# i8run/BigDL

Hardware: AMD Instinct MI355X
Metric: images/sec (whole node) ResNet-50 224x224 bf16 at 1/2/4/8 MI355X (higher is better)
Workload: dtype bf16; 1 GPU; model=ResNet-50 v1.5 (BigDL ImageNet builder), global_batch=256, per_gpu_batch=256, image=224, parallelism=dp1, optimizer=SGD momentum 0.9 + L2 1e-4 (one rank: no gradient exchange), hip_graph=False, wgrad_side_stream=True, bucketed_overlap=False, grad_compress=none (no exchange)

## Files before the change

### csrc/bindings.cpp

```cpp
#include <torch/extension.h>
#include <ATen/hip/HIPContext.h>
#include <vector>
#include <algorithm>
#include "kernels.h"

namespace {

using at::Tensor;
using OptT = c10::optional<Tensor>;

hipStream_t stream() { return at::hip::getCurrentHIPStream().stream(); }

void check(const Tensor& t, at::ScalarType dt, const char* name) {
  TORCH_CHECK(t.is_cuda(), name, " must be a GPU tensor");
  TORCH_CHECK(t.scalar_type() == dt, name, " has dtype ", t.scalar_type(), ", expected ", dt);
}
const uint16_t* cbf(const Tensor& t, const char* n) { check(t, at::kBFloat16, n); return (const uint16_t*)t.data_ptr(); }
uint16_t* mbf(const Tensor& t, const char* n) { check(t, at::kBFloat16, n); return (uint16_t*)t.data_ptr(); }
const float* cf(const Tensor& t, const char* n) { check(t, at::kFloat, n); return (const float*)t.data_ptr(); }
float* mf(const Tensor& t, const char* n) { check(t, at::kFloat, n); return (float*)t.data_ptr(); }
const uint16_t* ocbf(const OptT& t, const char* n) { return (t && t->defined()) ? cbf(*t, n) : nullptr; }
uint16_t* ombf(const OptT& t, const char* n) { return (t && t->defined()) ? mbf(*t, n) : nullptr; }
const float* ocf(const OptT& t, const char* n) { return (t && t->defined()) ? cf(*t, n) : nullptr; }
float* omf(const OptT& t, const char* n) { return (t && t->defined()) ? mf(*t, n) : nullptr; }
// ... 257 lines not shown
  TORCH_CHECK(geo.size() == 18, who, ": bad geometry");
  WgradArgs a{};
  int* f = &a.Nb;
  for (int i = 0; i < 18; ++i) f[i] = (int)geo[i];
  static float dummy;
  a.dbias = bias ? &dummy : nullptr;
  return bigdl_conv_wgrad_choose(&a);
}

bool conv_wgrad_uses_p8(std::vector<int64_t> geo, bool bias) {
  const int k = wgrad_choice_of(geo, bias, "conv_wgrad_uses_p8").kernel;
  return k == WGRAD_P8 || k == WGRAD_P8_DIRECT;
}

std::vector<int64_t> conv_wgrad_plan_info(std::vector<int64_t> geo, bool bias) {
  const WgradChoice c = wgrad_choice_of(geo, bias, "conv_wgrad_plan_info");
  const bool atomic = c.kernel == WGRAD_GLDS_ATOMIC || c.kernel == WGRAD_G3_ATOMIC;
  return {c.kernel == WGRAD_REG ? 0 : atomic ? 1 : c.splits, c.ws_floats, c.kernel == WGRAD_HALO ? c.splits : 0,
          c.kernel == WGRAD_P8 || c.kernel == WGRAD_P8_DIRECT, c.kernel == WGRAD_REG};
}

std::string conv_wgrad_plan_name(std::vector<int64_t> geo, bool bias) {
  return bigdl_wgrad_kernel_name(wgrad_choice_of(geo, bias, "conv_wgrad_plan_name").kernel);
}

void transpose_krsc(const Tensor& w, const Tensor& wt, int64_t K, int64_t RS, int64_t C) {
  TORCH_CHECK(w.numel() == K * RS * C && wt.numel() == K * RS * C, "transpose_krsc: size mismatch");
  bigdl_transpose_krsc(cbf(w, "w"), mbf(wt, "wt"), (int)K, (int)RS, (int)C, stream());
}

void bn_stats(const Tensor& x, const Tensor& stats, int64_t P, int64_t C) {
  TORCH_CHECK(C % 8 == 0 && x.numel() == P * C, "bn_stats: shape");
  TORCH_CHECK(stats.numel() >= BIGDL_STAT_SLOTS * 2 * C, "bn_stats: stats must hold STAT_SLOTS x 2C");
  bigdl_bn_stats(cbf(x, "x"), mf(stats, "stats"), P, (int)C, stream());
}
void bn_finalize(const Tensor& stats, int64_t nslots, const OptT& gamma, const OptT& beta, const OptT& rmean,
                 const OptT& rvar, const OptT& smean, const OptT& sinv, const Tensor& scale, const Tensor& shift,
                 int64_t P, int64_t C, double eps, double momentum, bool training) {
  TORCH_CHECK(stats.numel() >= nslots * 2 * C, "bn_finalize: stats size");
  bigdl_bn_finalize(cf(stats, "stats"), (int)nslots, ocf(gamma, "gamma"), ocf(beta, "beta"), omf(rmean, "rmean"),
                    omf(rvar, "rvar"), omf(smean, "smean"), omf(sinv, "sinv"), mf(scale, "scale"),
                    mf(shift, "shift"), P, (int)C, (float)eps, (float)momentum, training ? 1 : 0, stream());
}
void bn_slot_reduce(const Tensor& in, int64_t nslots, int64_t C, const Tensor& out) {
  TORCH_CHECK(in.numel() >= nslots * 2 * C && out.numel() >= 2 * C, "bn_slot_reduce: size");
  bigdl_bn_slot_reduce(cf(in, "in"), (int)nslots, (int)C, mf(out, "out"), stream());
// ... 1824 lines not shown
  m.def("set_conv_p8", &bigdl_set_conv_p8);
  m.def("set_conv_w8", &bigdl_set_conv_w8);
  m.def("set_wgrad_p8", &bigdl_set_wgrad_p8);
  m.def("conv_wgrad_uses_p8", &conv_wgrad_uses_p8);
  m.def("conv_wgrad_plan_info", &conv_wgrad_plan_info);
  m.def("conv_wgrad_plan_name", &conv_wgrad_plan_name);
  m.def("get_conv_shortk", &bigdl_get_conv_shortk);
  m.def("get_conv_p8", &bigdl_get_conv_p8);
  m.def("get_conv_w8", &bigdl_get_conv_w8);
  m.def("get_conv_sk", &bigdl_get_conv_sk);
  m.def("get_conv_s1", &bigdl_get_conv_s1);
  m.def("get_wgrad_p8", &bigdl_get_wgrad_p8);
  m.def("get_conv_halo", &bigdl_get_conv_halo);
  m.def("get_stem_fwd", &bigdl_get_stem_fwd);
  m.def("get_stem_wgrad", &bigdl_get_stem_wgrad);
  m.def("get_wgrad_halo", &bigdl_get_wgrad_halo);
  m.def("conv_nt_plan_info", &conv_nt_plan_info, py::arg("geo"), py::arg("taps"), py::arg("flags") = 0,
        py::arg("addend_stride") = std::vector<int64_t>());
  m.def("get_conv_g4", &bigdl_get_conv_g4);
  m.def("set_wgrad_g3", &bigdl_set_wgrad_g3);
  m.def("get_wgrad_g3", &bigdl_get_wgrad_g3);
  m.def("set_wgrad_tr_asm", &bigdl_set_wgrad_tr_asm);
  m.def("get_wgrad_tr_asm", &bigdl_get_wgrad_tr_asm);
  m.def("set_i8_g3", &bigdl_set_i8_g3);
  m.def("set_i8_p8", &bigdl_set_i8_p8);
  m.def("set_i8_s1", &bigdl_set_i8_s1);
  m.def("set_i8_epi", &bigdl_set_i8_epi);
  m.def("set_i8_shortk", &bigdl_set_i8_shortk);
  m.def("set_i8_cpl", &bigdl_set_i8_cpl);
  m.def("get_i8_g3", &bigdl_get_i8_g3);
  m.def("get_i8_p8", &bigdl_get_i8_p8);
  m.def("get_i8_s1", &bigdl_get_i8_s1);
  m.def("get_i8_epi", &bigdl_get_i8_epi);
  m.def("get_i8_shortk", &bigdl_get_i8_shortk);
  m.def("get_i8_cpl", &bigdl_get_i8_cpl);
  m.def("conv_i8_plan_info", &conv_i8_plan_info, py::arg("geo"), py::arg("taps"), py::arg("out_mode") = 0,
        py::arg("flags") = 0, py::arg("ldo_override") = 0, py::arg("add_ld") = 0,
        "(kernel, BM, BN, stages, cpl, direct, fastk) conv_i8 would run; launches nothing");
  m.attr("arch") = "gfx950";
}
```

### csrc/conv_igemm.hip

```cpp
#include "common.h"
#include "kernels.h"
#include <stdlib.h>

#include "conv_epilogue.h"
#include "lds_tr.h"


namespace {

constexpr int BK = 64;

__device__ __attribute__((aligned(64))) bf16_t g_zero_granule[32];
__device__ __forceinline__ v4u load16(const bf16_t* p, bool ok) {
  return *reinterpret_cast<const v4u*>(ok ? p : g_zero_granule);
}

template <int MI, int NI, int TM, int TN>
__device__ __forceinline__ void nt_epilogue(const ConvArgs& a, v4f (&acc)[MI][NI], int mbase, int nbase, int lane,
                                            int bid) {
  const int ohw = a.OH * a.OW;
  const bool vec_ok = (a.Ncol & 3) == 0 && (a.ldo & 3) == 0;
#pragma unroll
  for (int j = 0; j < NI; ++j) {
    const int nb = nbase + j * 16 + (lane >> 4) * 4;
// ... 2776 lines not shown
  const int tiles = ((a->Ncol + WT - 1) / WT) * ((a->Kdim + WT - 1) / WT);
  const bool dma = s.impl >= 1 && !wgrad_prefers_atomic(a);
  if (dma) {
    int splits = (s.wgrad_wgs + tiles - 1) / tiles;
    splits = std::max(1, std::min(splits, (a->M + 8 * WBM - 1) / (8 * WBM)));
    wgrad_split(&c, a->M, splits);
    if (c.splits > 1) {
      c.kernel = s.wgrad_g3 ? WGRAD_G3_WS : WGRAD_GLDS_WS;
      c.ws_floats = (long)c.splits * a->Ncol * a->Kdim;
      return c;
    }
  }
  int splits = (512 + tiles - 1) / tiles;
  const long tile_bytes = (long)tiles * WT * WT * 4;
  splits = std::min(splits, (int)(((long)s.wgrad_atomic_mb << 20) / tile_bytes));
  splits = std::min(splits, (a->M + 4 * WBM - 1) / (4 * WBM));
  if (splits < 1 || bigdl_deterministic()) splits = 1;
  wgrad_split(&c, a->M, splits);
  c.kernel = !dma ? WGRAD_REG : s.wgrad_g3 ? WGRAD_G3_ATOMIC : WGRAD_GLDS_ATOMIC;
  return c;
}

void launch_wgrad_reduce(const WgradArgs& a, int groups, hipStream_t st) {
  const long n4 = (long)a.Ncol * a.Kdim / 4;
  const int blocks = (int)std::min<long>((n4 + 255) / 256, 8192);
  if (groups < 0)
    groups = (blocks >= 256 || bigdl_deterministic()) ? 1 : std::max(1, std::min({2048 / blocks, a.splits / 4, 64}));
  const dim3 grid(blocks, groups);
  if ((reinterpret_cast<uintptr_t>(a.dw) & 15) == 0) wgrad_reduce_kernel<true><<<grid, 256, 0, st>>>(a.ws, a.dw, n4, a.splits);
  else wgrad_reduce_kernel<false><<<grid, 256, 0, st>>>(a.ws, a.dw, n4, a.splits);
}

}

extern "C" {

void bigdl_set_conv_impl(int v) { sw().impl = v; }
void bigdl_set_conv_s1(int v) { sw().s1 = v; }
void bigdl_set_conv_sk(int v) { sw().sk = v; }
void bigdl_set_conv_g4(int v) { sw().g4 = v; }
void bigdl_set_conv_shortk(int v) { sw().shortk = v; }
void bigdl_set_conv_p8(int v) { sw().p8 = v; }
void bigdl_set_conv_w8(int v) { sw().w8 = v; }
void bigdl_set_wgrad_p8(int v) { sw().wgrad_p8 = v; }
void bigdl_set_wgrad_g3(int v) { sw().wgrad_g3 = v; }
void bigdl_set_wgrad_tr_asm(int v) { sw().wgrad_tr_asm = v; }
// ... 183 lines not shown
      } else {
        if (direct) conv_wgrad_p8_kernel<true, false><<<grid, dim3(512), 0, st>>>(a);
        else conv_wgrad_p8_kernel<false, false><<<grid, dim3(512), 0, st>>>(a);
      }
      if (a.splits > 1) launch_wgrad_reduce(a, 1, st);
      break;
    }
    case WGRAD_GLDS_WS:
    case WGRAD_G3_WS:
      if (c->kernel == WGRAD_G3_WS) launch_wgrad_g3(a, tiles * spad, st);
      else launch_wgrad_glds(a, tiles * spad, st);
      launch_wgrad_reduce(a, -1, st);
      break;
    case WGRAD_GLDS_ATOMIC: launch_wgrad_glds(a, tiles * spad, st); break;
    case WGRAD_G3_ATOMIC: launch_wgrad_g3(a, tiles * spad, st); break;
    case WGRAD_REG: conv_wgrad_kernel<<<dim3(tiles, a.splits), dim3(256), 0, st>>>(a); break;
    default: return WGRAD_ERR_LAUNCH;
  }
  HIP_LAUNCH_CHECK();
  if (det_bias) bigdl_colsum_bf16_ld(a_in->dy, a_in->dbias, a_in->M, a_in->Ncol, a_in->ldy, st, a_in->det_ws);
  return 0;
}

void bigdl_transpose_krsc(const bf16_t* w, bf16_t* wt, int K, int RS, int C, hipStream_t st) {
  if (RS > 65535) return;
  if (K % 8 == 0 && C % 8 == 0 && (long)K * C >= (1L << 20) && (((uintptr_t)w | (uintptr_t)wt) & 15) == 0)
    transpose_krsc_v8_kernel<<<dim3((C + 63) / 64, (K + 63) / 64, RS), 256, 0, st>>>(w, wt, K, RS, C);
  else
    transpose_krsc_kernel<<<dim3((C + 31) / 32, (K + 31) / 32, RS), 256, 0, st>>>(w, wt, K, RS, C);
  HIP_LAUNCH_CHECK();
}

void bigdl_transpose_krsc_batched(const long* desc, int n, int total_tiles, hipStream_t st) {
  if (n <= 0 || total_tiles <= 0) return;
  transpose_krsc_batched_kernel<<<dim3(total_tiles), 256, 0, st>>>(desc, n);
  HIP_LAUNCH_CHECK();
}

}
```

### csrc/kernels.h

```cpp
#pragma once
#include <hip/hip_runtime.h>
#include <stdint.h>

#define CONV_MAX_TAPS 64
struct ConvArgs {
  const uint16_t* src;
  const uint16_t* wt;
  uint16_t* out;
  const float* bias;
  float* stats;
  const uint16_t* addend;
  const uint8_t* addzm;
  const uint16_t* bnx;
  const uint16_t* bnz;
  const uint8_t* bnzm;
  const float* bnmean;
  const float* bnaff;
  float* bnred;
  int Nb, Hs, Ws, Cs;
  int OH, OW;
  int mul_h, mul_w;
  int ntaps, ldw;
  int M, Ncol, Kdim, ldo;
  int OHo, OWo, omul_h, omul_w, ooff_h, ooff_w, ident_out;
// ... 185 lines not shown
                        const uint16_t* x2 = nullptr, const float* mean2 = nullptr, float* red2 = nullptr);

void bigdl_relu_fwd(const uint16_t* x, uint16_t* y, long n, hipStream_t st);
void bigdl_spin_us(double us, int* done, hipStream_t st);
void bigdl_dgrad_fill(uint16_t* out, const uint16_t* add, long npix, int H, int W, int C, int sh, int sw, unsigned mask,
                      hipStream_t st);
void bigdl_relu_bwd(const uint16_t* dy, const uint16_t* y, uint16_t* dx, long n, hipStream_t st);
void bigdl_add_bf16(const uint16_t* a, const uint16_t* b, uint16_t* y, long n, hipStream_t st);
void bigdl_nchw_f32_to_nhwc_bf16(const float* x, uint16_t* y, int N, int C, int H, int W, int Cp,
                                 hipStream_t st);
void bigdl_cast_f32_bf16(const float* x, uint16_t* y, long n, hipStream_t st);
void bigdl_colsum_bf16(const uint16_t* x, float* out, long P, int K, hipStream_t st, float* det_ws = nullptr);
void bigdl_ones_col_pack(const uint16_t* x, uint16_t* xe, long M, int K, hipStream_t st);
void bigdl_ones_col_acc(const float* gw, float* gW, float* gB, long N, int K, float sW, float sB, hipStream_t st);
void bigdl_cast_bf16_f32(const uint16_t* x, float* y, long n, hipStream_t st);

void bigdl_maxpool_fwd(const uint16_t* x, uint16_t* y, uint8_t* idx, int N, int H, int W, int C, int OH,
                       int OW, int kh, int kw, int sh, int sw, int ph, int pw, hipStream_t st, const float* pre = nullptr);
int bigdl_maxpool_pre_applies(int N, int H, int W, int C, int OH, int OW, int kh, int kw, int sh, int sw);
int bigdl_stem_i8_applies(const ConvArgs* a, const I8Epi* ep);
void bigdl_set_stem_i8(int v);
int bigdl_stem_i8_f32(const ConvArgs* a, const I8Epi* ep, const float* img, int C, int W, float inv, hipStream_t st);
int bigdl_stem_i8(const ConvArgs* a, const I8Epi* ep, hipStream_t st);
void bigdl_split_reduce_f32(const float* ws, float* dw, long n, int splits, hipStream_t st);
int bigdl_maxpool_bwd_bnred_applies(int N, int H, int W, int C, int OH, int OW, int kh, int kw, int sh, int sw, int ph,
                                    int pw);
void bigdl_maxpool_bwd_bnred(const uint16_t* dy, const uint8_t* idx, uint16_t* dx, int N, int C, int OH, int OW,
                             const uint16_t* bx, const float* mean, const float* aff, const uint8_t* zm, float* red,
                             hipStream_t st);
void bigdl_maxpool_bwd(const uint16_t* dy, const uint8_t* idx, uint16_t* dx, int N, int H, int W, int C,
                       int OH, int OW, int kh, int kw, int sh, int sw, int ph, int pw, hipStream_t st);
void bigdl_avgpool_fwd(const uint16_t* x, uint16_t* y, int N, int H, int W, int C, int OH, int OW, int kh,
                       int kw, int sh, int sw, int ph, int pw, int count_pad, hipStream_t st);
void bigdl_avgpool_bwd(const uint16_t* dy, uint16_t* dx, int N, int H, int W, int C, int OH, int OW, int kh,
                       int kw, int sh, int sw, int ph, int pw, int count_pad, hipStream_t st);

void bigdl_softmax_xent(const uint16_t* logits_bf16, const float* logits_f32, const float* labels,
                        float* loss, uint16_t* dlogits_bf16, float* dlogits_f32, int B, int K,
                        float label_base, float grad_scale, hipStream_t st, float* det_ws = nullptr);
#define BIGDL_XENT_SLOTS 2048

void bigdl_sgd_step(float* w, const float* g, float* mom, uint16_t* w16, long n, const float* lr_dev, float lr,
                    float wd, float momentum, double dampening, int nesterov, int first, const long* seg_off,
                    const float* seg_wd, int nseg, long base, hipStream_t st);
void bigdl_adam_step(float* w, const float* g, float* m, float* v, uint16_t* w16, long n, float lr,
                     double beta1, double beta2, float eps, float wd, float bc1, float bc2, hipStream_t st);
void bigdl_sumsq(const float* x, float* out, long n, hipStream_t st, float* det_ws = nullptr);
// ... 21 lines not shown
int bigdl_tensor_apply(float* out, const float* a, const float* b, const float* c, int nd, const long* size,
                       const long* so, const long* sa, const long* sb, const long* sc, int op, float s0, float s1,
                       int contiguous, hipStream_t st);
int bigdl_index_op(int op, float* a, const void* idx, int idx_i64, const float* b, float* out, long outer, long R,
                   long n, long inner, long Rsrc, int* err, hipStream_t st);
void bigdl_masked_fill(float* x, const float* mask, float v, long n, hipStream_t st);
long bigdl_mask_blocks(long n);
void bigdl_mask_scan(const float* mask, long n, int* counts, hipStream_t st);
void bigdl_mask_write(int copy, float* x, const float* mask, const float* src, float* out, long n, const int* counts,
                      long nsrc, hipStream_t st);
int bigdl_topk(const float* x, long outer, long R, long inner, int k, int largest, float* vals, float* inds,
               hipStream_t st);
int bigdl_tensor_reduce(const float* x, long outer, long R, long inner, int op, float p, float* out, float* outi,
                        int mean, float* ws, long chunks, hipStream_t st);
int bigdl_gemm_f32(const float* A, const float* B, const float* Min, float* C, int batch, int M, int N, int K,
                   const long* s, float alpha, float beta, hipStream_t st);
int bigdl_gemv_f32(const float* A, const float* x, const float* Min, float* y, int M, int K, long sam, long sak,
                   long sx, long smi, long sy, float alpha, float beta, hipStream_t st);
void bigdl_copy_rows_i8(const int8_t* src, int8_t* dst, long rows, int C, long lds, long ldd, hipStream_t st);
void bigdl_set_conv_impl(int impl);
void bigdl_set_conv_s1(int v);
void bigdl_set_conv_sk(int v);
void bigdl_set_wgrad_halo(int v);
int bigdl_lstm_drop_rep(const void* x, int x_bf16, long xs_b, long xs_t, uint16_t* y, long ys_g, int B, int T, int K,
                        int Kp, int ones, float p, float mul, unsigned long long seed, long long off, hipStream_t st);
int bigdl_lstm_drop_rep_bwd(const float* dy, long dys_g, int ldy, float* dx, long dxs_b, long dxs_t, const float* add,
                            long as_b, long as_t, int B, int T, int K, float p, float mul, unsigned long long seed,
                            long long off, hipStream_t st);
void bigdl_lstm_pack_gate_w(const float* W, const float* b1, const float* b2, int H, int Kin, int Kp, uint16_t* out,
                            uint16_t* outT, hipStream_t st);
int bigdl_wgrad_halo_plan(WgradArgs* a);
int bigdl_wgrad_pre_applies(const WgradArgs* a);
int bigdl_wgrad_halo(const WgradArgs* a, hipStream_t st);
int bigdl_get_conv_impl();
void bigdl_set_conv_g4(int v);
void bigdl_set_conv_shortk(int v);
void bigdl_set_conv_p8(int v);
void bigdl_set_conv_w8(int v);
void bigdl_set_wgrad_p8(int v);
int bigdl_get_conv_g4();
void bigdl_set_wgrad_g3(int v);
int bigdl_get_wgrad_g3();
void bigdl_set_wgrad_tr_asm(int v);
int bigdl_get_wgrad_tr_asm();
void bigdl_set_i8_g3(int v);
void bigdl_set_i8_p8(int v);
// ... 204 lines not shown
```

### csrc/stem_fwd.hip

```cpp
#include <algorithm>
#include <cstdlib>
#include <type_traits>
#include <utility>

#include "common.h"
#include "kernels.h"
#include "conv_epilogue.h"

namespace {

constexpr int SR = 7, SRB = 4, SOW = 112, SFM = SOW / 16, SXROWS = 2 * SRB + SR - 2;
constexpr int SWST = 30 * 16;

template <int WQ>
struct StemL {
  static constexpr int XB = SXROWS * WQ * 16;
  static constexpr int XG = (XB / 16 + 255) / 256;
  static constexpr int WOFF = (XG * 256 * 16 + 1023) / 1024 * 1024;
  static constexpr int LDS0 = WOFF + 64 * SWST;
  static constexpr int EPI = 4 * SFM * 16 * 128 + 4 * 128 * 4;
  static constexpr int LDS = LDS0 > EPI ? LDS0 : EPI;
};

struct StemRowMap {
// ... 295 lines not shown
  }
  return cus;
}

long bigdl_stem_wgrad_plan(const WgradArgs* a) {
  if (!bigdl_get_stem_wgrad() || a->Cs != 8 || a->R != SR || a->S != 4 || a->sh != 2 || a->sw != 1 || a->ph || a->pw ||
      a->dh != 1 || a->dwl != 1 || a->OW != SOW || a->Ws != 115 || (a->OH % SWRB) || a->Ncol != 64 ||
      a->Kdim != SR * 32 || a->ldy != 64 || a->M != a->Nb * a->OH * a->OW || a->Hs < 2 * a->OH + SR - 2)
    return 0;
  if ((size_t)a->Nb * a->Hs * a->Ws * 16 >= (1ull << 31) || (size_t)a->M * 128 >= (1ull << 31)) return 0;
  const long tiles = (long)a->Nb * (a->OH / SWRB);
  return (long)std::min<long>(tiles, stem_wgrad_grid()) * (64 * 224 + 64);
}

int bigdl_stem_wgrad(const WgradArgs* a, hipStream_t st) {
  const long tiles = (long)a->Nb * (a->OH / SWRB);
  const int grid = (int)std::min<long>(tiles, stem_wgrad_grid());
  if (a->pre_x) {
    if (!a->pre_coef || !a->pre_aff) return -7;
    stem_wgrad_kernel<115, true><<<dim3(grid), dim3(448), 0, st>>>(*a);
  } else {
    stem_wgrad_kernel<115, false><<<dim3(grid), dim3(448), 0, st>>>(*a);
  }
  bigdl_split_reduce_f32(a->ws, a->dw, 64 * 224, grid, st);
  if (a->dbias) bigdl_split_reduce_f32(a->ws + (size_t)grid * 64 * 224, a->dbias, 64, grid, st);
  return 0;
}

}
```

### csrc/wgrad_halo.hip

```cpp
#include <algorithm>
#include <cstdlib>
#include <type_traits>
#include <utility>

#include "common.h"
#include "kernels.h"

namespace {

__device__ __forceinline__ int hf128(int r) { return 2 * (((r >> 1) & 1) | (((r >> 3) & 1) << 1)); }
__device__ __forceinline__ int hf256(int r) { return 2 * ((r & 3) | (((r >> 3) & 1) << 2)); }

template <int W, int RB, int KB, int LDSKB>
struct Halo {
  static constexpr int WP = W + 2;
  static constexpr int V = (RB * WP + 31) / 32 * 32;
  static constexpr int NCH = V / 32;
  static constexpr int NW = KB / 16;
  static constexpr int NT = 64 * NW;
  static constexpr int XROWS = V + 2 * WP + 2;
  static constexpr int XG = (XROWS * 8 + NT - 1) / NT;
  static constexpr int XR = XG * NT / 8;
  static constexpr int DG = V * KB / 8 / NT;
  static constexpr int DROW = KB * 2;
// ... 22 lines not shown
template <class F, int... I>
__device__ __forceinline__ void sfor_impl(F&& f, std::integer_sequence<int, I...>) {
  (f(std::integral_constant<int, I>{}), ...);
}
template <int N, class F>
__device__ __forceinline__ void sfor(F&& f) {
  sfor_impl(f, std::make_integer_sequence<int, N>{});
}

template <int N>
__device__ __forceinline__ void vm_wait() {
  static_assert(N >= 0 && N < 64, "vmcnt range");
  asm volatile("s_waitcnt vmcnt(%0)" ::"n"(N) : "memory");
}
template <int D, int MAXK>
__device__ __forceinline__ void vm_wait_stages(int k) {
  if constexpr (MAXK >= 4) { if (k >= 4) { vm_wait<4 * D>(); return; } }
  if constexpr (MAXK >= 3) { if (k == 3) { vm_wait<3 * D>(); return; } }
  if constexpr (MAXK >= 2) { if (k == 2) { vm_wait<2 * D>(); return; } }
  if constexpr (MAXK >= 1) { if (k == 1) { vm_wait<D>(); return; } }
  vm_wait<0>();
}

template <int W, int RB, int KB, int LDSKB, bool PRE = false>
__global__ __launch_bounds__(KB * 4, 1) void conv_wgrad_halo_kernel(WgradArgs a) {
  using H = Halo<W, RB, KB, LDSKB>;
  __shared__ __attribute__((aligned(1024))) unsigned char lds[H::NS * H::STAGE + (PRE ? 512 : 0)];

  const int tid = threadIdx.x, lane = tid & 63;
  const int wave = __builtin_amdgcn_readfirstlane(tid >> 6);
  const int cw = wave & 3, kg = wave >> 2;
  const int C = a.Cs, K = a.Ncol, IH = a.Hs;
  const int tiles_c = C / 64, ntile = tiles_c * (K / KB);
  const int L = blockIdx.x, kq = L >> 3;
  const int split = 8 * (kq / ntile) + (L & 7);
  const int t = kq % ntile;
  const int c0 = (t % tiles_c) * 64, k0 = (t / tiles_c) * KB;
  const int spi = IH / RB, nstage_all = a.Nb * spi;
  const int st0 = split * a.m_per_split;
  const int nst = min(nstage_all, st0 + a.m_per_split) - st0;
  if (split >= a.splits || nst <= 0) return;

  constexpr unsigned OOB = 0x7ffffff0u;
  unsigned xv[4][H::XG];
#pragma unroll
  for (int d = 0; d < H::XG; ++d) {
    const int slot = (d * H::NW + wave) * 64 + lane;
    const int row = slot >> 3;
    const int g = (slot & 7) ^ hf128(row);
    const int xr = row - 1;
    const int rr = xr >= 0 ? xr / H::WP : -1, j = xr - rr * H::WP;
    const bool ok = xr >= 0 && rr < RB + 2 && j >= 1 && j <= W;
    const unsigned off = (unsigned)((rr * W + (j - 1)) * C + c0 + g * 8) * 2u;
#pragma unroll
    for (int v = 0; v < 4; ++v) {
      const bool bad = ((v & 1) && rr == 0) || ((v & 2) && rr == RB + 1);
      xv[v][d] = (ok && !bad) ? off : OOB;
    }
  }
  unsigned dv[H::DG];
#pragma unroll
  for (int d = 0; d < H::DG; ++d) {
    const int slot = (d * H::NW + wave) * 64 + lane;
    const int row = slot / (KB / 8);
    const int g = (slot % (KB / 8)) ^ (KB == 128 ? hf256(row) : hf128(row));
    const int rr = row / H::WP, j = row - rr * H::WP;
    const bool ok = rr < RB && j >= 1 && j <= W;
    dv[d] = ok ? (unsigned)((rr * W + (j - 1)) * a.ldy + k0 + g * 8) * 2u : OOB;
  }
  const bf16_t* xsrc = reinterpret_cast<const bf16_t*>(a.src);
  const bf16_t* dsrc = reinterpret_cast<const bf16_t*>(a.dy);
  const size_t xend = (size_t)a.Nb * IH * W * C, dend = (size_t)(a.M - 1) * a.ldy + K;

  float* const ptab = reinterpret_cast<float*>(lds + H::NS * H::STAGE);
  if constexpr (PRE) {
    if (tid < 32) {
      const int h = tid >> 4, i = tid & 15;
      reinterpret_cast<v4f*>(ptab)[tid] = reinterpret_cast<const v4f*>(a.pre + h * C + c0)[i];
    }
    __syncthreads();
  }
  int nx = st0 / spi, ohx = (st0 - nx * spi) * RB;
  auto issue = [&](int buf) {
    const int n = nx, oh0 = ohx;
    ohx += RB;
    if (ohx == IH) { ohx = 0; ++nx; }
    const size_t pix = ((size_t)n * IH + oh0) * W;
    const size_t xo = pix * C - (size_t)W * C;
    const __amdgpu_buffer_rsrc_t rx = __builtin_amdgcn_make_buffer_rsrc(
        const_cast<bf16_t*>(xsrc + xo), (short)0, (int)((xend - xo) * 2), 0x00020000);
    const __amdgpu_buffer_rsrc_t rd = __builtin_amdgcn_make_buffer_rsrc(
        const_cast<bf16_t*>(dsrc + pix * a.ldy), (short)0, (int)((dend - pix * a.ldy) * 2), 0x00020000);
    unsigned char* X = lds + buf * H::STAGE;
    const int v = (oh0 == 0 ? 1 : 0) | (oh0 + RB == IH ? 2 : 0);
    auto xdma = [&](auto vc) {
      constexpr int V = decltype(vc)::value;
#pragma unroll
      for (int d = 0; d < H::XG; ++d)
        __builtin_amdgcn_raw_ptr_buffer_load_lds(rx, (LDS_PTR(void))(X + (d * H::NW + wave) * 64 * 16), 16,
                                                 (int)xv[V][d], 0, 0, 0);
    };
    switch (v) {
      case 0: xdma(std::integral_constant<int, 0>{}); break;
      case 1: xdma(std::integral_constant<int, 1>{}); break;
      case 2: xdma(std::integral_constant<int, 2>{}); break;
      default: xdma(std::integral_constant<int, 3>{}); break;
    }
    unsigned char* Dt = X + H::XBYTES;
#pragma unroll
    for (int d = 0; d < H::DG; ++d)
      __builtin_amdgcn_raw_ptr_buffer_load_lds(rd, (LDS_PTR(void))(Dt + (d * H::NW + wave) * 64 * 16), 16,
                                               (int)dv[d], 0, 0, 0);
  };

  const int G = lane >> 4, q = (lane & 15) >> 2, p = lane & 3;
  int xa[9][2], da[4][2];
#pragma unroll
  for (int tp = 0; tp < 9; ++tp)
#pragma unroll
    for (int h = 0; h < 2; ++h) {
      const int row = 8 * G + q + 4 * h + (tp / 3) * H::WP + (tp % 3);
      xa[tp][h] = row * 128 + (((cw * 2 + (p >> 1)) ^ hf128(row)) << 4) + (p & 1) * 8;
    }
#pragma unroll
  for (int kb = 0; kb < 4; ++kb)
#pragma unroll
    for (int h = 0; h < 2; ++h) {
      const int row = 8 * G + q + 4 * h;
      const int gr = kg * 8 + kb * 2 + (p >> 1);
// ... 26 lines not shown
#pragma unroll
      for (int d0 = 0; d0 < H::XG; d0 += PG) {
        v4u u[PG];
        v4f s0[PG], s1[PG], b0[PG], b1[PG];
#pragma unroll
        for (int q = 0; q < PG; ++q) {
          const int d = d0 + q;
          if (d >= H::XG) break;
          const int slot = (d * H::NW + wave) * 64 + lane;
          const int g = (slot & 7) ^ hf128(slot >> 3);
          const unsigned ta = (unsigned)(uintptr_t)(LDS_PTR(float))ptab + (unsigned)(g * 32);
          const unsigned addr = xb + (unsigned)(slot * 16);
          asm volatile("ds_read_b128 %0, %5\n\tds_read_b128 %1, %6 offset:0\n\tds_read_b128 %2, %6 offset:16\n\t"
                       "ds_read_b128 %3, %6 offset:256\n\tds_read_b128 %4, %6 offset:272"
                       : "=v"(u[q]), "=v"(s0[q]), "=v"(s1[q]), "=v"(b0[q]), "=v"(b1[q]) : "v"(addr), "v"(ta) : "memory");
        }
        asm volatile("s_waitcnt lgkmcnt(0)" ::: "memory");
#pragma unroll
        for (int q = 0; q < PG; ++q) asm volatile("" : "+v"(u[q]), "+v"(s0[q]), "+v"(s1[q]), "+v"(b0[q]), "+v"(b1[q]));
#pragma unroll
        for (int q = 0; q < PG; ++q) {
          const int d = d0 + q;
          if (d >= H::XG) break;
          const unsigned off = v == 0 ? xv[0][d] : v == 1 ? xv[1][d] : v == 2 ? xv[2][d] : xv[3][d];
          const int slot = (d * H::NW + wave) * 64 + lane;
          const unsigned addr = xb + (unsigned)(slot * 16);
          const float sc[8] = {s0[q][0], s0[q][1], s0[q][2], s0[q][3], s1[q][0], s1[q][1], s1[q][2], s1[q][3]};
          const float sh[8] = {b0[q][0], b0[q][1], b0[q][2], b0[q][3], b1[q][0], b1[q][1], b1[q][2], b1[q][3]};
          v4u t;
#pragma unroll
          for (int e = 0; e < 4; ++e)
            t[e] = pack2bf(fmaxf(lo_bf(u[q][e]) * sc[2 * e] + sh[2 * e], 0.f),
                           fmaxf(hi_bf(u[q][e]) * sc[2 * e + 1] + sh[2 * e + 1], 0.f));
          const v4u o = off != OOB ? t : u[q];
          asm volatile("ds_write_b128 %0, %1" ::"v"(addr), "v"(o) : "memory");
        }
      }
      asm volatile("s_waitcnt lgkmcnt(0)" ::: "memory");
    }
    __builtin_amdgcn_s_barrier();
    asm volatile("" ::: "memory");
    if (i + H::NS - 1 < nst) issue((i + H::NS - 1) % H::NS);
    const unsigned sb = lds_base + (unsigned)((i % H::NS) * H::STAGE);
    unsigned xad[9][2], dad[4][2];
#pragma unroll
    for (int tp = 0; tp < 9; ++tp) { xad[tp][0] = sb + xa[tp][0]; xad[tp][1] = sb + xa[tp][1]; }
#pragma unroll
// ... 73 lines not shown
    int sp = g;
    for (; sp + 48 < splits; sp += 64) {
      const v4f a0 = w4[(long)sp * n4 + i], a1 = w4[(long)(sp + 16) * n4 + i];
      const v4f a2 = w4[(long)(sp + 32) * n4 + i], a3 = w4[(long)(sp + 48) * n4 + i];
      s0 += a0; s1 += a1; s2 += a2; s3 += a3;
    }
    for (; sp < splits; sp += 16) s0 += w4[(long)sp * n4 + i];
  }
  red[g][e] = (s0 + s1) + (s2 + s3);
  __syncthreads();
  if (g == 0 && i < n4) {
    v4f t = red[0][e];
#pragma unroll
    for (int r = 1; r < 16; ++r) t += red[r][e];
    if (aligned) {
      reinterpret_cast<v4f*>(dw)[i] += t;
    } else {
#pragma unroll
      for (int k = 0; k < 4; ++k) dw[4 * i + k] += t[k];
    }
  }
}

template <int W, int RB, int LDSKB>
void launch_halo(const WgradArgs& a, hipStream_t st) {
  const int ntile = (a.Cs / 64) * (a.Ncol / (a.Ncol % 128 == 0 ? 128 : 64));
  const int spad = (a.splits + 7) / 8 * 8;
  if (a.pre) {
    if constexpr (LDSKB <= 80) {
      if (a.Ncol % 128 == 0) conv_wgrad_halo_kernel<W, RB, 128, LDSKB, true><<<dim3(ntile * spad), dim3(512), 0, st>>>(a);
      else conv_wgrad_halo_kernel<W, RB, 64, LDSKB, true><<<dim3(ntile * spad), dim3(256), 0, st>>>(a);
    }
  } else if (a.Ncol % 128 == 0) {
    conv_wgrad_halo_kernel<W, RB, 128, LDSKB><<<dim3(ntile * spad), dim3(512), 0, st>>>(a);
  } else {
    conv_wgrad_halo_kernel<W, RB, 64, LDSKB><<<dim3(ntile * spad), dim3(256), 0, st>>>(a);
  }
}

template <int W, int RB>
void launch_halo_lds(const WgradArgs& a, int lds, hipStream_t st) {
  if (lds <= 80 || a.pre) launch_halo<W, RB, 80>(a, st);
  else launch_halo<W, RB, 160>(a, st);
}

int halo_rb(int W) { return W == 56 ? 1 : W == 28 ? 2 : W == 14 ? 2 : W == 7 ? 7 : 0; }

int g_wgrad_halo = -1;
int halo_lds() {
  static const int v = [] { const char* e = getenv("BIGDL_WGRAD_HALO_LDS"); return e ? atoi(e) : 80; }();
  return v;
}
bool halo_atomic() {
  static const int v = [] { const char* e = getenv("BIGDL_WGRAD_HALO_ATOMIC"); return e ? atoi(e) : 0; }();
  return v != 0 && !bigdl_deterministic();
}
int halo_wgs() {
  static const int v = [] { const char* e = getenv("BIGDL_WGRAD_HALO_WGS"); return e ? atoi(e) : 256; }();
  return v;
}

}

extern "C" {

void bigdl_set_wgrad_halo(int v) { g_wgrad_halo = v; }
int bigdl_get_wgrad_halo() {
  if (g_wgrad_halo < 0) {
    const char* e = getenv("BIGDL_WGRAD_HALO");
    g_wgrad_halo = e ? atoi(e) : 1;
  }
  return g_wgrad_halo;
}

int bigdl_wgrad_halo_plan(WgradArgs* a) {
  if (!bigdl_get_wgrad_halo()) return 0;
  const int rb = halo_rb(a->Ws);
  if (rb == 0 || a->R != 3 || a->S != 3 || a->sh != 1 || a->sw != 1 || a->ph != 1 || a->pw != 1 || a->dh != 1 ||
      a->dwl != 1 || a->OH != a->Hs || a->OW != a->Ws || (a->Hs % rb) || (a->Cs % 64) || (a->Ncol % 64) ||
      a->Kdim != 9 * a->Cs || a->ldy != a->Ncol || a->M != a->Nb * a->OH * a->OW || a->M <= 0)
    return 0;
  const long stages = (long)a->Nb * (a->Hs / rb);
  const int ntile = (a->Cs / 64) * (a->Ncol / (a->Ncol % 128 == 0 ? 128 : 64));
  const long x_bytes = (long)a->Nb * a->Hs * a->Ws * a->Cs * 2, dy_bytes = (long)a->M * a->ldy * 2;
  if (x_bytes >= (1L << 30) || dy_bytes >= (1L << 30)) return 0;
  long splits = std::max(1L, std::min(stages, ((long)halo_wgs() + ntile - 1) / ntile));
  const long sps = (stages + splits - 1) / splits;
  splits = (stages + sps - 1) / sps;
  a->m_per_split = (int)sps;
  return (int)splits;
}

int bigdl_wgrad_pre_applies(const WgradArgs* a) {
  WgradArgs b = *a;
  return bigdl_wgrad_halo_plan(&b) > 0 ? 1 : 0;
}

int bigdl_wgrad_halo(const WgradArgs* a_in, hipStream_t st) {
  const int lds = halo_lds();
  WgradArgs b = *a_in;
  if (b.splits > 1 && halo_atomic()) b.ws = nullptr;
  const WgradArgs* a = &b;
  switch (a->Ws) {
    case 56: launch_halo_lds<56, 1>(*a, lds, st); break;
    case 28: launch_halo_lds<28, 2>(*a, lds, st); break;
    case 14: launch_halo_lds<14, 2>(*a, lds, st); break;
    case 7: launch_halo_lds<7, 7>(*a, lds, st); break;
    default: return -1;
  }
  if (a->splits > 1 && a->ws != nullptr) {
    const long n4 = (long)a->Ncol * a->Kdim / 4;
    const int aligned = (reinterpret_cast<uintptr_t>(a->dw) & 15) == 0;
    halo_reduce_kernel<<<dim3((unsigned)((n4 + 15) / 16)), dim3(256), 0, st>>>(a->ws, a->dw, n4, a->splits, aligned);
    if (a->dbias)
      halo_reduce_kernel<<<dim3((unsigned)((a->Ncol / 4 + 15) / 16)), dim3(256), 0, st>>>(
          a->ws + (size_t)a->splits * a->Ncol * a->Kdim, a->dbias, a->Ncol / 4, a->splits,
          (reinterpret_cast<uintptr_t>(a->dbias) & 15) == 0);
  }
  return 0;
}

void bigdl_split_reduce_f32(const float* ws, float* dw, long n, int splits, hipStream_t st) {
  const long n4 = n / 4;
  halo_reduce_kernel<<<dim3((unsigned)((n4 + 15) / 16)), dim3(256), 0, st>>>(
      ws, dw, n4, splits, (reinterpret_cast<uintptr_t>(dw) & 15) == 0);
  HIP_LAUNCH_CHECK();
}

}
```

Before: 12530 images/sec.

## Add shape-adaptive split-sum reduction kernel for wgrad split workspaces

Replaces the split-K workspace reduction used by halo, stem and im2col wgrad paths with a new split_sum kernel. Its work-groups split the thread block across splits (SR) or across columns (NC) depending on split count, use non-temporal loads, and fold the bias reduction into the same launch. It also adds an optional flag-based halo offset scheme, off by default, that keeps fewer per-variant offset registers. The aim is to cut reduction-kernel time and launch count, at the cost of more template variants and an LDS cross-row reduction.

```diff
diff --git a/csrc/bindings.cpp b/csrc/bindings.cpp
--- a/csrc/bindings.cpp
+++ b/csrc/bindings.cpp
@@ -303,6 +303,20 @@
 
 std::string conv_wgrad_plan_name(std::vector<int64_t> geo, bool bias) {
   return bigdl_wgrad_kernel_name(wgrad_choice_of(geo, bias, "conv_wgrad_plan_name").kernel);
+}
+
+void split_reduce(const Tensor& ws, const Tensor& dw, int64_t n, int64_t splits, const OptT& dbias, int64_t nbias,
+                  bool im2col) {
+  float* db = omf(dbias, "dbias");
+  TORCH_CHECK(!(im2col && db), "split_reduce: the im2col launch has no bias block");
+  if (!db) nbias = 0;
+  TORCH_CHECK(n > 0 && n % 4 == 0 && nbias % 4 == 0 && splits >= 1 && splits < (1 << 30), "split_reduce: n and nbias are multiples of 4");
+  TORCH_CHECK(ws.is_contiguous() && ws.numel() >= splits * (n + nbias), "split_reduce: ws holds [splits][n] then [splits][nbias]");
+  TORCH_CHECK(dw.is_contiguous() && dw.numel() >= n, "split_reduce: dw too small");
+  TORCH_CHECK(!db || (dbias->is_contiguous() && dbias->numel() >= nbias), "split_reduce: dbias too small");
+  TORCH_CHECK((reinterpret_cast<uintptr_t>(ws.data_ptr()) & 15) == 0, "split_reduce: ws must be 16-byte aligned");
+  if (im2col) bigdl_wgrad_reduce_f32(mf(ws, "ws"), mf(dw, "dw"), n, (int)splits, stream());
+  else bigdl_split_reduce_f32(cf(ws, "ws"), mf(dw, "dw"), n, (int)splits, db, (int)nbias, stream());
 }
 
 void transpose_krsc(const Tensor& w, const Tensor& wt, int64_t K, int64_t RS, int64_t C) {
@@ -2173,6 +2187,14 @@
   m.def("get_wgrad_g3", &bigdl_get_wgrad_g3);
   m.def("set_wgrad_tr_asm", &bigdl_set_wgrad_tr_asm);
   m.def("get_wgrad_tr_asm", &bigdl_get_wgrad_tr_asm);
+  m.def("split_reduce", &split_reduce, py::arg("ws"), py::arg("dw"), py::arg("n"), py::arg("splits"),
+        py::arg("dbias") = py::none(), py::arg("nbias") = 0, py::arg("im2col") = false);
+  m.def("set_wgrad_halo_flags", &bigdl_set_wgrad_halo_flags);
+  m.def("get_wgrad_halo_flags", &bigdl_get_wgrad_halo_flags);
+  m.def("set_wgrad_split_sum", &bigdl_set_wgrad_split_sum);
+  m.def("get_wgrad_split_sum", &bigdl_get_wgrad_split_sum);
+  m.def("set_wgrad_split_sum_nt", &bigdl_set_wgrad_split_sum_nt);
+  m.def("get_wgrad_split_sum_nt", &bigdl_get_wgrad_split_sum_nt);
   m.def("set_i8_g3", &bigdl_set_i8_g3);
   m.def("set_i8_p8", &bigdl_set_i8_p8);
   m.def("set_i8_s1", &bigdl_set_i8_s1);
diff --git a/csrc/conv_igemm.hip b/csrc/conv_igemm.hip
--- a/csrc/conv_igemm.hip
+++ b/csrc/conv_igemm.hip
@@ -2822,6 +2822,10 @@
 }
 
 void launch_wgrad_reduce(const WgradArgs& a, int groups, hipStream_t st) {
+  if (bigdl_get_wgrad_split_sum()) {
+    bigdl_split_reduce_f32(a.ws, a.dw, (long)a.Ncol * a.Kdim, a.splits, nullptr, 0, st);
+    return;
+  }
   const long n4 = (long)a.Ncol * a.Kdim / 4;
   const int blocks = (int)std::min<long>((n4 + 255) / 256, 8192);
   if (groups < 0)
@@ -3051,6 +3055,13 @@
   return 0;
 }
 
+void bigdl_wgrad_reduce_f32(float* ws, float* dw, long n, int splits, hipStream_t st) {
+  WgradArgs a{};
+  a.ws = ws; a.dw = dw; a.Ncol = 4; a.Kdim = (int)(n / 4); a.splits = splits;
+  launch_wgrad_reduce(a, -1, st);
+  HIP_LAUNCH_CHECK();
+}
+
 void bigdl_transpose_krsc(const bf16_t* w, bf16_t* wt, int K, int RS, int C, hipStream_t st) {
   if (RS > 65535) return;
   if (K % 8 == 0 && C % 8 == 0 && (long)K * C >= (1L << 20) && (((uintptr_t)w | (uintptr_t)wt) & 15) == 0)
diff --git a/csrc/kernels.h b/csrc/kernels.h
--- a/csrc/kernels.h
+++ b/csrc/kernels.h
@@ -231,7 +231,12 @@
 void bigdl_set_stem_i8(int v);
 int bigdl_stem_i8_f32(const ConvArgs* a, const I8Epi* ep, const float* img, int C, int W, float inv, hipStream_t st);
 int bigdl_stem_i8(const ConvArgs* a, const I8Epi* ep, hipStream_t st);
-void bigdl_split_reduce_f32(const float* ws, float* dw, long n, int splits, hipStream_t st);
+void bigdl_split_reduce_f32(const float* ws, float* dw, long n, int splits, float* dbias, int nbias, hipStream_t st);
+void bigdl_wgrad_reduce_f32(float* ws, float* dw, long n, int splits, hipStream_t st);
+void bigdl_set_wgrad_split_sum(int v);
+int bigdl_get_wgrad_split_sum();
+void bigdl_set_wgrad_split_sum_nt(int v);
+int bigdl_get_wgrad_split_sum_nt();
 int bigdl_maxpool_bwd_bnred_applies(int N, int H, int W, int C, int OH, int OW, int kh, int kw, int sh, int sw, int ph,
                                     int pw);
 void bigdl_maxpool_bwd_bnred(const uint16_t* dy, const uint8_t* idx, uint16_t* dx, int N, int C, int OH, int OW,
@@ -299,6 +304,8 @@
 void bigdl_set_conv_s1(int v);
 void bigdl_set_conv_sk(int v);
 void bigdl_set_wgrad_halo(int v);
+void bigdl_set_wgrad_halo_flags(int v);
+int bigdl_get_wgrad_halo_flags();
 int bigdl_lstm_drop_rep(const void* x, int x_bf16, long xs_b, long xs_t, uint16_t* y, long ys_g, int B, int T, int K,
                         int Kp, int ones, float p, float mul, unsigned long long seed, long long off, hipStream_t st);
 int bigdl_lstm_drop_rep_bwd(const float* dy, long dys_g, int ldy, float* dx, long dxs_b, long dxs_t, const float* add,
diff --git a/csrc/stem_fwd.hip b/csrc/stem_fwd.hip
--- a/csrc/stem_fwd.hip
+++ b/csrc/stem_fwd.hip
@@ -341,8 +341,7 @@
   } else {
     stem_wgrad_kernel<115, false><<<dim3(grid), dim3(448), 0, st>>>(*a);
   }
-  bigdl_split_reduce_f32(a->ws, a->dw, 64 * 224, grid, st);
-  if (a->dbias) bigdl_split_reduce_f32(a->ws + (size_t)grid * 64 * 224, a->dbias, 64, grid, st);
+  bigdl_split_reduce_f32(a->ws, a->dw, 64 * 224, grid, a->dbias, a->dbias ? 64 : 0, st);
   return 0;
 }
 
diff --git a/csrc/wgrad_halo.hip b/csrc/wgrad_halo.hip
--- a/csrc/wgrad_halo.hip
+++ b/csrc/wgrad_halo.hip
@@ -68,7 +68,7 @@
   vm_wait<0>();
 }
 
-template <int W, int RB, int KB, int LDSKB, bool PRE = false>
+template <int W, int RB, int KB, int LDSKB, bool PRE = false, bool FL = false>
 __global__ __launch_bounds__(KB * 4, 1) void conv_wgrad_halo_kernel(WgradArgs a) {
   using H = Halo<W, RB, KB, LDSKB>;
   __shared__ __attribute__((aligned(1024))) unsigned char lds[H::NS * H::STAGE + (PRE ? 512 : 0)];
@@ -88,7 +88,7 @@
   if (split >= a.splits || nst <= 0) return;
 
   constexpr unsigned OOB = 0x7ffffff0u;
-  unsigned xv[4][H::XG];
+  unsigned xv[4][H::XG], xo[H::XG], xfl = 0;
 #pragma unroll
   for (int d = 0; d < H::XG; ++d) {
     const int slot = (d * H::NW + wave) * 64 + lane;
@@ -98,12 +98,22 @@
     const int rr = xr >= 0 ? xr / H::WP : -1, j = xr - rr * H::WP;
     const bool ok = xr >= 0 && rr < RB + 2 && j >= 1 && j <= W;
     const unsigned off = (unsigned)((rr * W + (j - 1)) * C + c0 + g * 8) * 2u;
-#pragma unroll
-    for (int v = 0; v < 4; ++v) {
-      const bool bad = ((v & 1) && rr == 0) || ((v & 2) && rr == RB + 1);
-      xv[v][d] = (ok && !bad) ? off : OOB;
-    }
-  }
+    if constexpr (FL) {
+      xo[d] = ok ? off : OOB;
+      if (ok && rr == 0) xfl |= 1u << d;
+      if (ok && rr == RB + 1) xfl |= 0x100u << d;
+    } else {
+#pragma unroll
+      for (int v = 0; v < 4; ++v) {
+        const bool bad = ((v & 1) && rr == 0) || ((v & 2) && rr == RB + 1);
+        xv[v][d] = (ok && !bad) ? off : OOB;
+      }
+    }
+  }
+  auto xoff = [&](int d, int v) {
+    const unsigned kill = xfl & ((v & 1 ? 0xffu : 0u) | (v & 2 ? 0xff00u : 0u));
+    return (kill & (0x101u << d)) ? OOB : xo[d];
+  };
   unsigned dv[H::DG];
 #pragma unroll
   for (int d = 0; d < H::DG; ++d) {
@@ -146,11 +156,18 @@
         __builtin_amdgcn_raw_ptr_buffer_load_lds(rx, (LDS_PTR(void))(X + (d * H::NW + wave) * 64 * 16), 16,
                                                  (int)xv[V][d], 0, 0, 0);
     };
-    switch (v) {
-      case 0: xdma(std::integral_constant<int, 0>{}); break;
-      case 1: xdma(std::integral_constant<int, 1>{}); break;
-      case 2: xdma(std::integral_constant<int, 2>{}); break;
-      default: xdma(std::integral_constant<int, 3>{}); break;
+    if constexpr (FL) {
+#pragma unroll
+      for (int d = 0; d < H::XG; ++d)
+        __builtin_amdgcn_raw_ptr_buffer_load_lds(rx, (LDS_PTR(void))(X + (d * H::NW + wave) * 64 * 16), 16,
+                                                 (int)xoff(d, v), 0, 0, 0);
+    } else {
+      switch (v) {
+        case 0: xdma(std::integral_constant<int, 0>{}); break;
+        case 1: xdma(std::integral_constant<int, 1>{}); break;
+        case 2: xdma(std::integral_constant<int, 2>{}); break;
+        default: xdma(std::integral_constant<int, 3>{}); break;
+      }
     }
     unsigned char* Dt = X + H::XBYTES;
 #pragma unroll
@@ -223,7 +240,9 @@
         for (int q = 0; q < PG; ++q) {
           const int d = d0 + q;
           if (d >= H::XG) break;
-          const unsigned off = v == 0 ? xv[0][d] : v == 1 ? xv[1][d] : v == 2 ? xv[2][d] : xv[3][d];
+          unsigned off;
+          if constexpr (FL) off = xoff(d, v);
+          else off = v == 0 ? xv[0][d] : v == 1 ? xv[1][d] : v == 2 ? xv[2][d] : xv[3][d];
           const int slot = (d * H::NW + wave) * 64 + lane;
           const unsigned addr = xb + (unsigned)(slot * 16);
           const float sc[8] = {s0[q][0], s0[q][1], s0[q][2], s0[q][3], s1[q][0], s1[q][1], s1[q][2], s1[q][3]};
@@ -343,26 +362,113 @@
   }
 }
 
-template <int W, int RB, int LDSKB>
+template <int SR, int NC, bool NT>
+__global__ __launch_bounds__(256) void split_sum_kernel(const float* __restrict__ ws, float* __restrict__ dw, long n4,
+                                                       int splits, int nwg_main, float* __restrict__ dbias, long nb4,
+                                                       int aligned) {
+  constexpr int CW = 256 / SR, U = 8 / NC;
+  __shared__ v4f red[SR > 1 ? SR : 1][SR > 1 ? CW + 1 : 1];
+  const v4f* w4 = reinterpret_cast<const v4f*>(ws);
+  float* out = dw;
+  long n = n4, wg = blockIdx.x;
+  bool al = aligned & 1;
+  if (wg >= nwg_main) {
+    wg -= nwg_main;
+    w4 += (long)splits * n4;
+    out = dbias;
+    n = nb4;
+    al = aligned & 2;
+  }
+  const int e = threadIdx.x % CW, g = threadIdx.x / CW;
+  const long col0 = wg * (CW * NC) + e;
+  const v4f zero = {0.f, 0.f, 0.f, 0.f};
+  v4f acc[NC];
+#pragma unroll
+  for (int j = 0; j < NC; ++j) acc[j] = zero;
+  for (int sp0 = g; sp0 < splits; sp0 += SR * U) {
+    v4f v[NC][U];
+#pragma unroll
+    for (int u = 0; u < U; ++u)
+#pragma unroll
+      for (int j = 0; j < NC; ++j) {
+        const int sp = sp0 + u * SR;
+        const long i = col0 + j * CW;
+        v[j][u] = zero;
+        if (sp < splits && i < n) {
+          const v4f* p = w4 + (long)sp * n + i;
+          v[j][u] = NT ? __builtin_nontemporal_load(p) : *p;
+        }
+      }
+#pragma unroll
+    for (int j = 0; j < NC; ++j) {
+#pragma unroll
+      for (int w = 1; w < U; w *= 2)
+#pragma unroll
+        for (int u = 0; u + w < U; u += 2 * w) v[j][u] += v[j][u + w];
+      acc[j] += v[j][0];
+    }
+  }
+  if constexpr (SR > 1) {
+    red[g][e] = acc[0];
+    __syncthreads();
+    if (g != 0) return;
+#pragma unroll 8
+    for (int r = 1; r < SR; ++r) acc[0] += red[r][e];
+  }
+#pragma unroll
+  for (int j = 0; j < NC; ++j) {
+    const long i = col0 + j * CW;
+    if (i >= n) continue;
+    if (al) {
+      reinterpret_cast<v4f*>(out)[i] += acc[j];
+    } else {
+#pragma unroll
+      for (int k = 0; k < 4; ++k) out[4 * i + k] += acc[j][k];
+    }
+  }
+}
+
+template <int SR, int NC>
+void launch_split_sum(const float* ws, float* dw, long n4, int splits, float* dbias, long nb4, bool nt, hipStream_t st) {
+  constexpr long COLS = 256 / SR * NC;
+  const long nwg_main = (n4 + COLS - 1) / COLS, nwg_bias = dbias ? (nb4 + COLS - 1) / COLS : 0;
+  const int aligned = ((reinterpret_cast<uintptr_t>(dw) & 15) == 0 ? 1 : 0) |
+                      ((reinterpret_cast<uintptr_t>(dbias) & 15) == 0 ? 2 : 0);
+  const dim3 grid((unsigned)(nwg_main + nwg_bias));
+  if (nt) split_sum_kernel<SR, NC, true><<<grid, dim3(256), 0, st>>>(ws, dw, n4, splits, (int)nwg_main, dbias, nb4, aligned);
+  else split_sum_kernel<SR, NC, false><<<grid, dim3(256), 0, st>>>(ws, dw, n4, splits, (int)nwg_main, dbias, nb4, aligned);
+}
+
+int g_split_sum = -1, g_split_sum_nt = -1;
+
+template <int W, int RB, int LDSKB, bool FL>
 void launch_halo(const WgradArgs& a, hipStream_t st) {
   const int ntile = (a.Cs / 64) * (a.Ncol / (a.Ncol % 128 == 0 ? 128 : 64));
   const int spad = (a.splits + 7) / 8 * 8;
   if (a.pre) {
     if constexpr (LDSKB <= 80) {
-      if (a.Ncol % 128 == 0) conv_wgrad_halo_kernel<W, RB, 128, LDSKB, true><<<dim3(ntile * spad), dim3(512), 0, st>>>(a);
-      else conv_wgrad_halo_kernel<W, RB, 64, LDSKB, true><<<dim3(ntile * spad), dim3(256), 0, st>>>(a);
+      if (a.Ncol % 128 == 0) conv_wgrad_halo_kernel<W, RB, 128, LDSKB, true, FL><<<dim3(ntile * spad), dim3(512), 0, st>>>(a);
+      else conv_wgrad_halo_kernel<W, RB, 64, LDSKB, true, FL><<<dim3(ntile * spad), dim3(256), 0, st>>>(a);
     }
   } else if (a.Ncol % 128 == 0) {
-    conv_wgrad_halo_kernel<W, RB, 128, LDSKB><<<dim3(ntile * spad), dim3(512), 0, st>>>(a);
+    conv_wgrad_halo_kernel<W, RB, 128, LDSKB, false, FL><<<dim3(ntile * spad), dim3(512), 0, st>>>(a);
   } else {
-    conv_wgrad_halo_kernel<W, RB, 64, LDSKB><<<dim3(ntile * spad), dim3(256), 0, st>>>(a);
-  }
-}
+    conv_wgrad_halo_kernel<W, RB, 64, LDSKB, false, FL><<<dim3(ntile * spad), dim3(256), 0, st>>>(a);
+  }
+}
+
+int g_wgrad_halo_flags = -1;
 
 template <int W, int RB>
 void launch_halo_lds(const WgradArgs& a, int lds, hipStream_t st) {
-  if (lds <= 80 || a.pre) launch_halo<W, RB, 80>(a, st);
-  else launch_halo<W, RB, 160>(a, st);
+  const bool fl = bigdl_get_wgrad_halo_flags() != 0;
+  if (lds <= 80 || a.pre) {
+    if (fl) launch_halo<W, RB, 80, true>(a, st);
+    else launch_halo<W, RB, 80, false>(a, st);
+  } else {
+    if (fl) launch_halo<W, RB, 160, true>(a, st);
+    else launch_halo<W, RB, 160, false>(a, st);
+  }
 }
 
 int halo_rb(int W) { return W == 56 ? 1 : W == 28 ? 2 : W == 14 ? 2 : W == 7 ? 7 : 0; }
@@ -386,6 +492,14 @@
 extern "C" {
 
 void bigdl_set_wgrad_halo(int v) { g_wgrad_halo = v; }
+void bigdl_set_wgrad_halo_flags(int v) { g_wgrad_halo_flags = v; }
+int bigdl_get_wgrad_halo_flags() {
+  if (g_wgrad_halo_flags < 0) {
+    const char* e = getenv("BIGDL_WGRAD_HALO_FLAGS");
+    g_wgrad_halo_flags = e ? atoi(e) : 0;
+  }
+  return g_wgrad_halo_flags;
+}
 int bigdl_get_wgrad_halo() {
   if (g_wgrad_halo < 0) {
     const char* e = getenv("BIGDL_WGRAD_HALO");
@@ -429,22 +543,50 @@
     case 7: launch_halo_lds<7, 7>(*a, lds, st); break;
     default: return -1;
   }
-  if (a->splits > 1 && a->ws != nullptr) {
-    const long n4 = (long)a->Ncol * a->Kdim / 4;
-    const int aligned = (reinterpret_cast<uintptr_t>(a->dw) & 15) == 0;
-    halo_reduce_kernel<<<dim3((unsigned)((n4 + 15) / 16)), dim3(256), 0, st>>>(a->ws, a->dw, n4, a->splits, aligned);
-    if (a->dbias)
-      halo_reduce_kernel<<<dim3((unsigned)((a->Ncol / 4 + 15) / 16)), dim3(256), 0, st>>>(
-          a->ws + (size_t)a->splits * a->Ncol * a->Kdim, a->dbias, a->Ncol / 4, a->splits,
-          (reinterpret_cast<uintptr_t>(a->dbias) & 15) == 0);
-  }
+  if (a->splits > 1 && a->ws != nullptr)
+    bigdl_split_reduce_f32(a->ws, a->dw, (long)a->Ncol * a->Kdim, a->splits, a->dbias, a->dbias ? a->Ncol : 0, st);
   return 0;
 }
 
-void bigdl_split_reduce_f32(const float* ws, float* dw, long n, int splits, hipStream_t st) {
-  const long n4 = n / 4;
-  halo_reduce_kernel<<<dim3((unsigned)((n4 + 15) / 16)), dim3(256), 0, st>>>(
-      ws, dw, n4, splits, (reinterpret_cast<uintptr_t>(dw) & 15) == 0);
+void bigdl_set_wgrad_split_sum(int v) { g_split_sum = v; }
+int bigdl_get_wgrad_split_sum() {
+  if (g_split_sum < 0) {
+    const char* e = getenv("BIGDL_WGRAD_SPLIT_SUM");
+    g_split_sum = e ? atoi(e) : 1;
+  }
+  return g_split_sum;
+}
+void bigdl_set_wgrad_split_sum_nt(int v) { g_split_sum_nt = v; }
+int bigdl_get_wgrad_split_sum_nt() {
+  if (g_split_sum_nt < 0) {
+    const char* e = getenv("BIGDL_WGRAD_SPLIT_SUM_NT");
+    g_split_sum_nt = e ? atoi(e) : 1;
+  }
+  return g_split_sum_nt;
+}
+
+void bigdl_split_reduce_f32(const float* ws, float* dw, long n, int splits, float* dbias, int nbias, hipStream_t st) {
+  const long n4 = n / 4, nb4 = dbias ? nbias / 4 : 0;
+  if (!dbias || nb4 == 0) dbias = nullptr;
+  if (!bigdl_get_wgrad_split_sum()) {
+    halo_reduce_kernel<<<dim3((unsigned)((n4 + 15) / 16)), dim3(256), 0, st>>>(
+        ws, dw, n4, splits, (reinterpret_cast<uintptr_t>(dw) & 15) == 0);
+    if (dbias)
+      halo_reduce_kernel<<<dim3((unsigned)((nb4 + 15) / 16)), dim3(256), 0, st>>>(
+          ws + (size_t)splits * n, dbias, nb4, splits, (reinterpret_cast<uintptr_t>(dbias) & 15) == 0);
+    HIP_LAUNCH_CHECK();
+    return;
+  }
+  const bool nt = bigdl_get_wgrad_split_sum_nt() != 0;
+  if (splits >= 256 && n4 <= 8 * 2048) launch_split_sum<32, 1>(ws, dw, n4, splits, dbias, nb4, nt, st);
+  else if (splits >= 128) launch_split_sum<16, 1>(ws, dw, n4, splits, dbias, nb4, nt, st);
+  else if (splits >= 64) launch_split_sum<8, 1>(ws, dw, n4, splits, dbias, nb4, nt, st);
+  else if (splits >= 32) launch_split_sum<4, 1>(ws, dw, n4, splits, dbias, nb4, nt, st);
+  else if (splits >= 16) launch_split_sum<2, 1>(ws, dw, n4, splits, dbias, nb4, nt, st);
+  else if (splits >= 8) launch_split_sum<1, 1>(ws, dw, n4, splits, dbias, nb4, nt, st);
+  else if (splits >= 4) launch_split_sum<1, 2>(ws, dw, n4, splits, dbias, nb4, nt, st);
+  else if (splits >= 2) launch_split_sum<1, 4>(ws, dw, n4, splits, dbias, nb4, nt, st);
+  else launch_split_sum<1, 8>(ws, dw, n4, splits, dbias, nb4, nt, st);
   HIP_LAUNCH_CHECK();
 }
 
```

New measurement: 12340 images/sec. 1.5% lower.
